# One-2-3-45/One-2-3-45

Measured on NVIDIA H100. Metric: sec/mesh end-to-end (256x256 in), lower is better.
Workload: dtype f16

## Files before the change

### one-2-3-45_b200/csrc/attention.cu

```cuda
#include <cuda_fp16.h>

#include "common.cuh"
#include "mma_sync.cuh"

namespace o2345 {
namespace {

__device__ __forceinline__ float ex2(float x) {
  float y;
  asm("ex2.approx.ftz.f32 %0, %1;" : "=f"(y) : "f"(x));
  return y;
}

constexpr int KT = 64;

template <int D, int DP, int NW>
__global__ void __launch_bounds__(32 * NW)
attention_kernel(const __half* __restrict__ q, const __half* __restrict__ k, const __half* __restrict__ v, int N, int H, int ld,
                 __half* __restrict__ out, int ldo, float scale_log2) {
  pdl_wait();
  pdl_trigger();
  constexpr int QT = 16 * NW, NT = 32 * NW;
  constexpr int LDQ = DP + 8, KS = DP / 16, NO = DP / 8;
  constexpr int STAGE = 2 * KT * LDQ;
  extern __shared__ __align__(16) __half smem_h[];
  __half* sQ = smem_h;
  __half* sKV = sQ + QT * LDQ;
  const int tid = threadIdx.x, warp = tid >> 5, lane = tid & 31, g = lane >> 2, t = lane & 3;
  const int bh = blockIdx.y, b = bh / H, h = bh % H;
  const int q0 = blockIdx.x * QT;
  const int64_t base = (int64_t)b * N * ld + (int64_t)h * D;
  constexpr int CH = D / 8;

  auto load_tile = [&](int stage, int k0) {
    __half* dK = sKV + stage * STAGE;
    __half* dV = dK + KT * LDQ;
    for (int i = tid; i < KT * CH; i += NT) {
      const int r = i / CH, c = i % CH;
      const bool in = k0 + r < N;
      const int64_t off = base + (int64_t)(in ? k0 + r : 0) * ld + 8 * c;
      const uint32_t ak = (uint32_t)__cvta_generic_to_shared(dK + r * LDQ + 8 * c), av = (uint32_t)__cvta_generic_to_shared(dV + r * LDQ + 8 * c);
      asm volatile("cp.async.cg.shared.global [%0], [%1], 16;" ::"r"(ak), "l"(k + off) : "memory");
      asm volatile("cp.async.cg.shared.global [%0], [%1], 16, %2;" ::"r"(av), "l"(v + off), "r"(in ? 16 : 0) : "memory");
    }
    asm volatile("cp.async.commit_group;" ::: "memory");
  };

  for (int i = tid; i < (QT * LDQ + 2 * STAGE) / 8; i += NT) reinterpret_cast<uint4*>(sQ)[i] = make_uint4(0, 0, 0, 0);
  __syncthreads();
  load_tile(0, 0);
  for (int i = tid; i < QT * CH; i += NT) {
    int r = i / CH, c = i % CH;
    if (q0 + r < N) *reinterpret_cast<uint4*>(sQ + r * LDQ + 8 * c) = *reinterpret_cast<const uint4*>(q + base + (int64_t)(q0 + r) * ld + 8 * c);
  }
  __syncthreads();
  uint32_t qa[KS][4];
#pragma unroll
  for (int kk = 0; kk < KS; ++kk) {
    const __half* p0 = sQ + (16 * warp + g) * LDQ + 16 * kk + 2 * t;
    qa[kk][0] = *reinterpret_cast<const uint32_t*>(p0);
    qa[kk][1] = *reinterpret_cast<const uint32_t*>(p0 + 8 * LDQ);
    qa[kk][2] = *reinterpret_cast<const uint32_t*>(p0 + 8);
    qa[kk][3] = *reinterpret_cast<const uint32_t*>(p0 + 8 * LDQ + 8);
  }
  float o[NO][4];
#pragma unroll
  for (int n = 0; n < NO; ++n) o[n][0] = o[n][1] = o[n][2] = o[n][3] = 0.f;
  float m0 = -1e30f, m1 = -1e30f;
  float ls[4] = {0.f, 0.f, 0.f, 0.f};

  int it = 0;
  for (int k0 = 0; k0 < N; k0 += KT, ++it) {
    asm volatile("cp.async.wait_group 0;" ::: "memory");
    __syncthreads();
    if (k0 + KT < N) load_tile((it + 1) & 1, k0 + KT);
    const __half* sK = sKV + (it & 1) * STAGE;
    const __half* sV = sK + KT * LDQ;
    float s[KT / 8][4];
#pragma unroll
    for (int j = 0; j < KT / 8; j += 2) {
      s[j][0] = s[j][1] = s[j][2] = s[j][3] = 0.f;
      s[j + 1][0] = s[j + 1][1] = s[j + 1][2] = s[j + 1][3] = 0.f;
#pragma unroll
      for (int kk = 0; kk < KS; ++kk) {
        uint32_t b0, b1, b2, b3;
        const uint32_t addr = (uint32_t)__cvta_generic_to_shared(sK + (8 * j + 8 * (lane >> 4) + (lane & 7)) * LDQ + 16 * kk + 8 * ((lane >> 3) & 1));
        asm volatile("ldmatrix.sync.aligned.m8n8.x4.shared.b16 {%0, %1, %2, %3}, [%4];" : "=r"(b0), "=r"(b1), "=r"(b2), "=r"(b3) : "r"(addr));
        mma16816(s[j], qa[kk], b0, b1);
        mma16816(s[j + 1], qa[kk], b2, b3);
      }
    }
    if (k0 + KT > N) {
#pragma unroll
      for (int j = 0; j < KT / 8; ++j) {
        const int key = k0 + 8 * j + 2 * t;
        if (key >= N) s[j][0] = -1e30f, s[j][2] = -1e30f;
        if (key + 1 >= N) s[j][1] = -1e30f, s[j][3] = -1e30f;
      }
    }
    float mx0 = -1e30f, mx1 = -1e30f;
#pragma unroll
    for (int j = 0; j < KT / 8; ++j) {
      mx0 = fmaxf(mx0, fmaxf(s[j][0], s[j][1]));
      mx1 = fmaxf(mx1, fmaxf(s[j][2], s[j][3]));
    }
    mx0 = fmaxf(mx0, __shfl_xor_sync(0xffffffffu, mx0, 1)), mx0 = fmaxf(mx0, __shfl_xor_sync(0xffffffffu, mx0, 2));
    mx1 = fmaxf(mx1, __shfl_xor_sync(0xffffffffu, mx1, 1)), mx1 = fmaxf(mx1, __shfl_xor_sync(0xffffffffu, mx1, 2));
    const float mn0 = fmaxf(m0, mx0), mn1 = fmaxf(m1, mx1);
    const float a0 = ex2((m0 - mn0) * scale_log2), a1 = ex2((m1 - mn1) * scale_log2);
    m0 = mn0, m1 = mn1;
    const float ms0 = -mn0 * scale_log2, ms1 = -mn1 * scale_log2;
#pragma unroll
    for (int n = 0; n < NO; ++n) o[n][0] *= a0, o[n][1] *= a0, o[n][2] *= a1, o[n][3] *= a1;
    ls[0] *= a0, ls[1] *= a0, ls[2] *= a1, ls[3] *= a1;
#pragma unroll
    for (int kk = 0; kk < KT / 16; ++kk) {
      const uint32_t pa[4] = {pack2(ex2(fmaf(s[2 * kk][0], scale_log2, ms0)), ex2(fmaf(s[2 * kk][1], scale_log2, ms0))),
                              pack2(ex2(fmaf(s[2 * kk][2], scale_log2, ms1)), ex2(fmaf(s[2 * kk][3], scale_log2, ms1))),
                              pack2(ex2(fmaf(s[2 * kk + 1][0], scale_log2, ms0)), ex2(fmaf(s[2 * kk + 1][1], scale_log2, ms0))),
                              pack2(ex2(fmaf(s[2 * kk + 1][2], scale_log2, ms1)), ex2(fmaf(s[2 * kk + 1][3], scale_log2, ms1)))};
      mma16816(ls, pa, 0x3C003C00u, 0x3C003C00u);
#pragma unroll
      for (int n = 0; n < NO; ++n) {
        uint32_t b0, b1;
        const uint32_t addr = (uint32_t)__cvta_generic_to_shared(sV + (16 * kk + (lane & 15)) * LDQ + 8 * n);
        asm volatile("ldmatrix.sync.aligned.m8n8.x2.trans.shared.b16 {%0, %1}, [%2];" : "=r"(b0), "=r"(b1) : "r"(addr));
        mma16816(o[n], pa, b0, b1);
      }
    }
  }
  const float l0 = ls[0], l1 = ls[2];
  float i0 = 1.f / l0, i1 = 1.f / l1;
  int row0 = q0 + 16 * warp + g, row1 = row0 + 8;
#pragma unroll
  for (int n = 0; n < NO; ++n) {
    int col = 8 * n + 2 * t;
    if (col < D) {
      if (row0 < N) *reinterpret_cast<uint32_t*>(out + ((int64_t)b * N + row0) * ldo + h * D + col) = pack2(o[n][0] * i0, o[n][1] * i0);
      if (row1 < N) *reinterpret_cast<uint32_t*>(out + ((int64_t)b * N + row1) * ldo + h * D + col) = pack2(o[n][2] * i1, o[n][3] * i1);
    }
  }
}

}
}

using namespace o2345;

extern "C" int o2345_attention_f16(const void* q, const void* k, const void* v, int B, int N, int H, int d, int ld, void* out,
                                   int ldo, float scale, o2345_stream_t stream) {
  O2345_CHECK_ARG(q && k && v && out, "null pointer");
  O2345_CHECK_ARG(B > 0 && N > 0 && H > 0 && (ld % 8) == 0 && (ldo % 2) == 0, "bad sizes");
  O2345_CHECK_ARG(d == 40 || d == 64 || d == 80 || d == 160, "head dim must be 40, 64, 80 or 160");
  O2345_CHECK_ARG(((uintptr_t)q % 16) == 0 && ((uintptr_t)k % 16) == 0 && ((uintptr_t)v % 16) == 0, "q/k/v must be 16-byte aligned");
  const int nw = N >= 512 ? 8 : 4;
  dim3 grid(cdiv(N, 16 * nw), B * H);
  float sl2 = scale * 1.4426950408889634f;
  cudaStream_t st = (cudaStream_t)stream;
  const __half *qh = (const __half*)q, *kh = (const __half*)k, *vh = (const __half*)v;
  auto smem = [&](int dp) { return (size_t)((16 * nw + 4 * KT) * (dp + 8)) * sizeof(__half); };
  static PerDeviceOnce attr;
  if (attr.need()) {
    O2345_CUDA(cudaFuncSetAttribute(attention_kernel<160, 160, 4>, cudaFuncAttributeMaxDynamicSharedMemorySize, (int)((64 + 4 * KT) * 168 * 2)));
    O2345_CUDA(cudaFuncSetAttribute(attention_kernel<160, 160, 8>, cudaFuncAttributeMaxDynamicSharedMemorySize, (int)((128 + 4 * KT) * 168 * 2)));
    O2345_CUDA(cudaFuncSetAttribute(attention_kernel<80, 80, 4>, cudaFuncAttributeMaxDynamicSharedMemorySize, (int)((64 + 4 * KT) * 88 * 2)));
    O2345_CUDA(cudaFuncSetAttribute(attention_kernel<80, 80, 8>, cudaFuncAttributeMaxDynamicSharedMemorySize, (int)((128 + 4 * KT) * 88 * 2)));
    O2345_CUDA(cudaFuncSetAttribute(attention_kernel<64, 64, 8>, cudaFuncAttributeMaxDynamicSharedMemorySize, (int)((128 + 4 * KT) * 72 * 2)));
  }
#define O2345_ATT(D_, DP_)                                                                                                        \
  do {                                                                                                                            \
    if (nw == 8)                                                                                                                  \
      O2345_CUDA(launch_pdl(attention_kernel<D_, DP_, 8>, dim3(grid), dim3(256), smem(DP_), st, qh, kh, vh, N, H, ld, (__half*)out, \
                            ldo, sl2));                                                                                           \
    else                                                                                                                          \
      O2345_CUDA(launch_pdl(attention_kernel<D_, DP_, 4>, dim3(grid), dim3(128), smem(DP_), st, qh, kh, vh, N, H, ld, (__half*)out, \
                            ldo, sl2));                                                                                           \
  } while (0)
  if (d == 40) O2345_ATT(40, 48);
  else if (d == 64) O2345_ATT(64, 64);
  else if (d == 80) O2345_ATT(80, 80);
  else if (d == 160) O2345_ATT(160, 160);
  else { set_error("o2345_attention_f16: head dim %d not built (40 / 64 / 80 / 160)", d); return O2345_EUNSUPPORTED; }
#undef O2345_ATT
  O2345_LAUNCH_CHECK();
  return O2345_OK;
}
```

### one-2-3-45_b200/csrc/wgmma.cuh

```cuda
#pragma once
#include <stdint.h>

namespace o2345 {
namespace wg {

__device__ __forceinline__ uint64_t desc_sw128(uint32_t saddr) {
  uint64_t d = 0;
  d |= (uint64_t)((saddr >> 4) & 0x3FFF);
  d |= (uint64_t)1 << 16;
  d |= (uint64_t)(1024 >> 4) << 32;
  d |= (uint64_t)1 << 62;
  return d;
}
__device__ __forceinline__ void fence() { asm volatile("wgmma.fence.sync.aligned;" ::: "memory"); }
__device__ __forceinline__ void commit() { asm volatile("wgmma.commit_group.sync.aligned;" ::: "memory"); }
template <int N>
__device__ __forceinline__ void wait() { asm volatile("wgmma.wait_group.sync.aligned %0;" ::"n"(N) : "memory"); }

template <int N>
__device__ __forceinline__ void mma_f16(float (&d)[N / 2], uint64_t adesc, uint64_t bdesc, int accumulate);

template <>
__device__ __forceinline__ void mma_f16<16>(float (&d)[8], uint64_t adesc, uint64_t bdesc, int accumulate) {
  asm volatile(
      "{\n\t.reg .pred p;\n\tsetp.ne.b32 p, %10, 0;\n\t"
      "wgmma.mma_async.sync.aligned.m64n16k16.f32.f16.f16 {%0, %1, %2, %3, %4, %5, %6, %7}, %8, %9, p, 1, 1, 0, 0;\n\t}"
      : "+f"(d[0]), "+f"(d[1]), "+f"(d[2]), "+f"(d[3]), "+f"(d[4]), "+f"(d[5]), "+f"(d[6]), "+f"(d[7])
      : "l"(adesc), "l"(bdesc), "r"(accumulate));
}

template <>
__device__ __forceinline__ void mma_f16<32>(float (&d)[16], uint64_t adesc, uint64_t bdesc, int accumulate) {
  asm volatile(
      "{\n\t.reg .pred p;\n\tsetp.ne.b32 p, %18, 0;\n\t"
      "wgmma.mma_async.sync.aligned.m64n32k16.f32.f16.f16 {%0, %1, %2, %3, %4, %5, %6, %7, %8, %9, %10, %11, %12, %13, %14, %15}, %16, %17, p, 1, 1, 0, 0;\n\t}"
      : "+f"(d[0]), "+f"(d[1]), "+f"(d[2]), "+f"(d[3]), "+f"(d[4]), "+f"(d[5]), "+f"(d[6]), "+f"(d[7]), "+f"(d[8]), "+f"(d[9]), "+f"(d[10]), "+f"(d[11]), "+f"(d[12]), "+f"(d[13]), "+f"(d[14]), "+f"(d[15])
      : "l"(adesc), "l"(bdesc), "r"(accumulate));
}

template <>
__device__ __forceinline__ void mma_f16<48>(float (&d)[24], uint64_t adesc, uint64_t bdesc, int accumulate) {
  asm volatile(
      "{\n\t.reg .pred p;\n\tsetp.ne.b32 p, %26, 0;\n\t"
      "wgmma.mma_async.sync.aligned.m64n48k16.f32.f16.f16 {%0, %1, %2, %3, %4, %5, %6, %7, %8, %9, %10, %11, %12, %13, %14, %15, %16, %17, %18, %19, %20, %21, %22, %23}, %24, %25, p, 1, 1, 0, 0;\n\t}"
      : "+f"(d[0]), "+f"(d[1]), "+f"(d[2]), "+f"(d[3]), "+f"(d[4]), "+f"(d[5]), "+f"(d[6]), "+f"(d[7]), "+f"(d[8]), "+f"(d[9]), "+f"(d[10]), "+f"(d[11]), "+f"(d[12]), "+f"(d[13]), "+f"(d[14]), "+f"(d[15]), "+f"(d[16]), "+f"(d[17]), "+f"(d[18]), "+f"(d[19]), "+f"(d[20]), "+f"(d[21]), "+f"(d[22]), "+f"(d[23])
      : "l"(adesc), "l"(bdesc), "r"(accumulate));
}

template <>
__device__ __forceinline__ void mma_f16<64>(float (&d)[32], uint64_t adesc, uint64_t bdesc, int accumulate) {
  asm volatile(
      "{\n\t.reg .pred p;\n\tsetp.ne.b32 p, %34, 0;\n\t"
      "wgmma.mma_async.sync.aligned.m64n64k16.f32.f16.f16 {%0, %1, %2, %3, %4, %5, %6, %7, %8, %9, %10, %11, %12, %13, %14, %15, %16, %17, %18, %19, %20, %21, %22, %23, %24, %25, %26, %27, %28, %29, %30, %31}, %32, %33, p, 1, 1, 0, 0;\n\t}"
      : "+f"(d[0]), "+f"(d[1]), "+f"(d[2]), "+f"(d[3]), "+f"(d[4]), "+f"(d[5]), "+f"(d[6]), "+f"(d[7]), "+f"(d[8]), "+f"(d[9]), "+f"(d[10]), "+f"(d[11]), "+f"(d[12]), "+f"(d[13]), "+f"(d[14]), "+f"(d[15]), "+f"(d[16]), "+f"(d[17]), "+f"(d[18]), "+f"(d[19]), "+f"(d[20]), "+f"(d[21]), "+f"(d[22]), "+f"(d[23]), "+f"(d[24]), "+f"(d[25]), "+f"(d[26]), "+f"(d[27]), "+f"(d[28]), "+f"(d[29]), "+f"(d[30]), "+f"(d[31])
      : "l"(adesc), "l"(bdesc), "r"(accumulate));
}

template <>
__device__ __forceinline__ void mma_f16<128>(float (&d)[64], uint64_t adesc, uint64_t bdesc, int accumulate) {
  asm volatile(
      "{\n\t.reg .pred p;\n\tsetp.ne.b32 p, %66, 0;\n\t"
      "wgmma.mma_async.sync.aligned.m64n128k16.f32.f16.f16 {%0, %1, %2, %3, %4, %5, %6, %7, %8, %9, %10, %11, %12, %13, %14, %15, %16, %17, %18, %19, %20, %21, %22, %23, %24, %25, %26, %27, %28, %29, %30, %31, %32, %33, %34, %35, %36, %37, %38, %39, %40, %41, %42, %43, %44, %45, %46, %47, %48, %49, %50, %51, %52, %53, %54, %55, %56, %57, %58, %59, %60, %61, %62, %63}, %64, %65, p, 1, 1, 0, 0;\n\t}"
      : "+f"(d[0]), "+f"(d[1]), "+f"(d[2]), "+f"(d[3]), "+f"(d[4]), "+f"(d[5]), "+f"(d[6]), "+f"(d[7]), "+f"(d[8]), "+f"(d[9]), "+f"(d[10]), "+f"(d[11]), "+f"(d[12]), "+f"(d[13]), "+f"(d[14]), "+f"(d[15]), "+f"(d[16]), "+f"(d[17]), "+f"(d[18]), "+f"(d[19]), "+f"(d[20]), "+f"(d[21]), "+f"(d[22]), "+f"(d[23]), "+f"(d[24]), "+f"(d[25]), "+f"(d[26]), "+f"(d[27]), "+f"(d[28]), "+f"(d[29]), "+f"(d[30]), "+f"(d[31]), "+f"(d[32]), "+f"(d[33]), "+f"(d[34]), "+f"(d[35]), "+f"(d[36]), "+f"(d[37]), "+f"(d[38]), "+f"(d[39]), "+f"(d[40]), "+f"(d[41]), "+f"(d[42]), "+f"(d[43]), "+f"(d[44]), "+f"(d[45]), "+f"(d[46]), "+f"(d[47]), "+f"(d[48]), "+f"(d[49]), "+f"(d[50]), "+f"(d[51]), "+f"(d[52]), "+f"(d[53]), "+f"(d[54]), "+f"(d[55]), "+f"(d[56]), "+f"(d[57]), "+f"(d[58]), "+f"(d[59]), "+f"(d[60]), "+f"(d[61]), "+f"(d[62]), "+f"(d[63])
      : "l"(adesc), "l"(bdesc), "r"(accumulate));
}

template <>
__device__ __forceinline__ void mma_f16<160>(float (&d)[80], uint64_t adesc, uint64_t bdesc, int accumulate) {
  asm volatile(
      "{\n\t.reg .pred p;\n\tsetp.ne.b32 p, %82, 0;\n\t"
      "wgmma.mma_async.sync.aligned.m64n160k16.f32.f16.f16 {%0, %1, %2, %3, %4, %5, %6, %7, %8, %9, %10, %11, %12, %13, %14, %15, %16, %17, %18, %19, %20, %21, %22, %23, %24, %25, %26, %27, %28, %29, %30, %31, %32, %33, %34, %35, %36, %37, %38, %39, %40, %41, %42, %43, %44, %45, %46, %47, %48, %49, %50, %51, %52, %53, %54, %55, %56, %57, %58, %59, %60, %61, %62, %63, %64, %65, %66, %67, %68, %69, %70, %71, %72, %73, %74, %75, %76, %77, %78, %79}, %80, %81, p, 1, 1, 0, 0;\n\t}"
      : "+f"(d[0]), "+f"(d[1]), "+f"(d[2]), "+f"(d[3]), "+f"(d[4]), "+f"(d[5]), "+f"(d[6]), "+f"(d[7]), "+f"(d[8]), "+f"(d[9]), "+f"(d[10]), "+f"(d[11]), "+f"(d[12]), "+f"(d[13]), "+f"(d[14]), "+f"(d[15]), "+f"(d[16]), "+f"(d[17]), "+f"(d[18]), "+f"(d[19]), "+f"(d[20]), "+f"(d[21]), "+f"(d[22]), "+f"(d[23]), "+f"(d[24]), "+f"(d[25]), "+f"(d[26]), "+f"(d[27]), "+f"(d[28]), "+f"(d[29]), "+f"(d[30]), "+f"(d[31]), "+f"(d[32]), "+f"(d[33]), "+f"(d[34]), "+f"(d[35]), "+f"(d[36]), "+f"(d[37]), "+f"(d[38]), "+f"(d[39]), "+f"(d[40]), "+f"(d[41]), "+f"(d[42]), "+f"(d[43]), "+f"(d[44]), "+f"(d[45]), "+f"(d[46]), "+f"(d[47]), "+f"(d[48]), "+f"(d[49]), "+f"(d[50]), "+f"(d[51]), "+f"(d[52]), "+f"(d[53]), "+f"(d[54]), "+f"(d[55]), "+f"(d[56]), "+f"(d[57]), "+f"(d[58]), "+f"(d[59]), "+f"(d[60]), "+f"(d[61]), "+f"(d[62]), "+f"(d[63]), "+f"(d[64]), "+f"(d[65]), "+f"(d[66]), "+f"(d[67]), "+f"(d[68]), "+f"(d[69]), "+f"(d[70]), "+f"(d[71]), "+f"(d[72]), "+f"(d[73]), "+f"(d[74]), "+f"(d[75]), "+f"(d[76]), "+f"(d[77]), "+f"(d[78]), "+f"(d[79])
      : "l"(adesc), "l"(bdesc), "r"(accumulate));
}

template <>
__device__ __forceinline__ void mma_f16<256>(float (&d)[128], uint64_t adesc, uint64_t bdesc, int accumulate) {
  asm volatile(
      "{\n\t.reg .pred p;\n\tsetp.ne.b32 p, %130, 0;\n\t"
      "wgmma.mma_async.sync.aligned.m64n256k16.f32.f16.f16 {%0, %1, %2, %3, %4, %5, %6, %7, %8, %9, %10, %11, %12, %13, %14, %15, %16, %17, %18, %19, %20, %21, %22, %23, %24, %25, %26, %27, %28, %29, %30, %31, %32, %33, %34, %35, %36, %37, %38, %39, %40, %41, %42, %43, %44, %45, %46, %47, %48, %49, %50, %51, %52, %53, %54, %55, %56, %57, %58, %59, %60, %61, %62, %63, %64, %65, %66, %67, %68, %69, %70, %71, %72, %73, %74, %75, %76, %77, %78, %79, %80, %81, %82, %83, %84, %85, %86, %87, %88, %89, %90, %91, %92, %93, %94, %95, %96, %97, %98, %99, %100, %101, %102, %103, %104, %105, %106, %107, %108, %109, %110, %111, %112, %113, %114, %115, %116, %117, %118, %119, %120, %121, %122, %123, %124, %125, %126, %127}, %128, %129, p, 1, 1, 0, 0;\n\t}"
      : "+f"(d[0]), "+f"(d[1]), "+f"(d[2]), "+f"(d[3]), "+f"(d[4]), "+f"(d[5]), "+f"(d[6]), "+f"(d[7]), "+f"(d[8]), "+f"(d[9]), "+f"(d[10]), "+f"(d[11]), "+f"(d[12]), "+f"(d[13]), "+f"(d[14]), "+f"(d[15]), "+f"(d[16]), "+f"(d[17]), "+f"(d[18]), "+f"(d[19]), "+f"(d[20]), "+f"(d[21]), "+f"(d[22]), "+f"(d[23]), "+f"(d[24]), "+f"(d[25]), "+f"(d[26]), "+f"(d[27]), "+f"(d[28]), "+f"(d[29]), "+f"(d[30]), "+f"(d[31]), "+f"(d[32]), "+f"(d[33]), "+f"(d[34]), "+f"(d[35]), "+f"(d[36]), "+f"(d[37]), "+f"(d[38]), "+f"(d[39]), "+f"(d[40]), "+f"(d[41]), "+f"(d[42]), "+f"(d[43]), "+f"(d[44]), "+f"(d[45]), "+f"(d[46]), "+f"(d[47]), "+f"(d[48]), "+f"(d[49]), "+f"(d[50]), "+f"(d[51]), "+f"(d[52]), "+f"(d[53]), "+f"(d[54]), "+f"(d[55]), "+f"(d[56]), "+f"(d[57]), "+f"(d[58]), "+f"(d[59]), "+f"(d[60]), "+f"(d[61]), "+f"(d[62]), "+f"(d[63]), "+f"(d[64]), "+f"(d[65]), "+f"(d[66]), "+f"(d[67]), "+f"(d[68]), "+f"(d[69]), "+f"(d[70]), "+f"(d[71]), "+f"(d[72]), "+f"(d[73]), "+f"(d[74]), "+f"(d[75]), "+f"(d[76]), "+f"(d[77]), "+f"(d[78]), "+f"(d[79]), "+f"(d[80]), "+f"(d[81]), "+f"(d[82]), "+f"(d[83]), "+f"(d[84]), "+f"(d[85]), "+f"(d[86]), "+f"(d[87]), "+f"(d[88]), "+f"(d[89]), "+f"(d[90]), "+f"(d[91]), "+f"(d[92]), "+f"(d[93]), "+f"(d[94]), "+f"(d[95]), "+f"(d[96]), "+f"(d[97]), "+f"(d[98]), "+f"(d[99]), "+f"(d[100]), "+f"(d[101]), "+f"(d[102]), "+f"(d[103]), "+f"(d[104]), "+f"(d[105]), "+f"(d[106]), "+f"(d[107]), "+f"(d[108]), "+f"(d[109]), "+f"(d[110]), "+f"(d[111]), "+f"(d[112]), "+f"(d[113]), "+f"(d[114]), "+f"(d[115]), "+f"(d[116]), "+f"(d[117]), "+f"(d[118]), "+f"(d[119]), "+f"(d[120]), "+f"(d[121]), "+f"(d[122]), "+f"(d[123]), "+f"(d[124]), "+f"(d[125]), "+f"(d[126]), "+f"(d[127])
      : "l"(adesc), "l"(bdesc), "r"(accumulate));
}

}
}
```

Measured before the change: 2.505.

## Add wgmma-based flash attention kernel for head dim 40

Adds a Hopper warpgroup-MMA attention kernel for head dimension 40. It uses a 4-stage cp.async K/V pipeline with core-matrix shared layouts, and overlaps the next tile's QK^T wgmma with the current tile's PV wgmma. The row sum is folded into the PV matmul by appending a ones column to V and a masking column to Q/K, which also masks out-of-range keys. This targets the mma.sync tensor-core throughput limit for the d=40 attention in the diffusion UNet, at the cost of more complex descriptor and layout logic and a higher risk of correctness bugs.

```diff
diff --git a/one-2-3-45_b200/csrc/attention.cu b/one-2-3-45_b200/csrc/attention.cu
--- a/one-2-3-45_b200/csrc/attention.cu
+++ b/one-2-3-45_b200/csrc/attention.cu
@@ -2,6 +2,7 @@
 
 #include "common.cuh"
 #include "mma_sync.cuh"
+#include "wgmma.cuh"
 
 namespace o2345 {
 namespace {
@@ -16,7 +17,7 @@
 
 template <int D, int DP, int NW>
 __global__ void __launch_bounds__(32 * NW)
-attention_kernel(const __half* __restrict__ q, const __half* __restrict__ k, const __half* __restrict__ v, int N, int H, int ld,
+attention_mma_kernel(const __half* __restrict__ q, const __half* __restrict__ k, const __half* __restrict__ v, int N, int H, int ld,
                  __half* __restrict__ out, int ldo, float scale_log2) {
   pdl_wait();
   pdl_trigger();
@@ -142,10 +143,175 @@
   }
 }
 
+template <int N>
+__device__ __forceinline__ void fence_regs(float (&r)[N]) {
+#pragma unroll
+  for (int i = 0; i < N; ++i) asm volatile("" : "+f"(r[i])::"memory");
+}
+
+constexpr int STAGES = 4;
+
+__device__ __forceinline__ uint32_t cm_off(int r, int c, int C) { return (uint32_t)((r >> 3) * (C * 128) + c * 128 + (r & 7) * 16); }
+
+template <int D, int NWG>
+struct AttCfg {
+  static constexpr int CH = D / 8;
+  static constexpr int CK = (CH + 2) / 2 * 2;
+  static constexpr int DV = D + 8;
+  static constexpr int CV = DV / 8;
+  static constexpr int QT = 64 * NWG;
+  static constexpr int QB = QT * CK * 16, KB = KT * CK * 16, VB = KT * CV * 16, SB = KB + VB;
+  static constexpr int SMEM = QB + STAGES * SB;
+};
+
+template <int D, int NWG>
+__global__ void __launch_bounds__(128 * NWG)
+attention_wgmma_kernel(const __half* __restrict__ q, const __half* __restrict__ k, const __half* __restrict__ v, int N, int H, int ld,
+                 __half* __restrict__ out, int ldo, float scale_log2) {
+  pdl_wait();
+  pdl_trigger();
+  using C = AttCfg<D, NWG>;
+  constexpr int CH = C::CH, CK = C::CK, CV = C::CV, DV = C::DV, NT = 128 * NWG;
+  extern __shared__ __align__(128) uint8_t smem[];
+  const uint32_t sbase = (uint32_t)__cvta_generic_to_shared(smem);
+  const int tid = threadIdx.x, warp = tid >> 5, lane = tid & 31, g = lane >> 2, t = lane & 3, wg = warp >> 2;
+  const int bh = blockIdx.y, b = bh / H, h = bh % H;
+  const int q0 = blockIdx.x * C::QT;
+  const int64_t base = (int64_t)b * N * ld + (int64_t)h * D;
+  const int nt = (N + KT - 1) / KT;
+
+  for (int i = tid; i < STAGES * KT; i += NT) {
+    uint8_t* st = smem + C::QB + (i / KT) * C::SB;
+    const int r = i % KT;
+    *reinterpret_cast<uint4*>(st + C::KB + cm_off(r, CH, CV)) = make_uint4(0x3C003C00u, 0x3C003C00u, 0x3C003C00u, 0x3C003C00u);
+#pragma unroll
+    for (int c = CH; c < CK; ++c) *reinterpret_cast<uint4*>(st + cm_off(r, c, CK)) = make_uint4(0, 0, 0, 0);
+  }
+  for (int i = tid; i < C::QT; i += NT)
+#pragma unroll
+    for (int c = CH; c < CK; ++c) *reinterpret_cast<uint4*>(smem + cm_off(i, c, CK)) = make_uint4(c == CH ? 0x3C00u : 0u, 0, 0, 0);
+
+  auto copy_rows = [&](uint32_t dst, int C_, const __half* src, int r0, int rows) {
+    for (int i = tid; i < rows * CH; i += NT) {
+      const int rr = i & 7, c = (i >> 3) % CH, r = (i >> 3) / CH * 8 + rr;
+      const bool in = r0 + r < N;
+      const __half* p = src + base + (int64_t)(in ? r0 + r : 0) * ld + 8 * c;
+      asm volatile("cp.async.cg.shared.global [%0], [%1], 16, %2;" ::"r"(dst + cm_off(r, c, C_)), "l"(p), "r"(in ? 16 : 0) : "memory");
+    }
+  };
+  auto load_tile = [&](int j) {
+    const uint32_t st = sbase + C::QB + (j % STAGES) * C::SB;
+    if (j < nt) {
+      copy_rows(st, CK, k, j * KT, KT);
+      copy_rows(st + C::KB, CV, v, j * KT, KT);
+    }
+    asm volatile("cp.async.commit_group;" ::: "memory");
+    if (j == nt - 1)
+      for (int r = N - j * KT + tid; r < KT; r += NT)
+        *reinterpret_cast<uint4*>(smem + (st - sbase) + cm_off(r, CH, CK)) = make_uint4(0xFC00u, 0, 0, 0);
+  };
+  copy_rows(sbase, CK, q, q0, C::QT);
+  load_tile(0);
+  load_tile(1);
+  load_tile(2);
+
+  const uint64_t qdesc = wg::desc_plain(sbase + wg * 64 * CK * 16, 128, CK * 128);
+  auto issue_s = [&](float (&s)[32], int j) {
+    const uint32_t st = sbase + C::QB + (j % STAGES) * C::SB;
+    fence_regs(s);
+    wg::fence();
+#pragma unroll
+    for (int kk = 0; kk < CK / 2; ++kk) wg::mma_f16<64>(s, qdesc + 16 * kk, wg::desc_plain(st + 256 * kk, 128, CK * 128), kk);
+    wg::commit();
+  };
+  float s[32], o[DV / 2];
+#pragma unroll
+  for (int i = 0; i < DV / 2; ++i) o[i] = 0.f;
+  float m0 = -1e30f, m1 = -1e30f;
+  float a0 = 1.f, a1 = 1.f;
+  uint32_t pa[KT / 16][4];
+
+  auto softmax = [&]() {
+    float mx0 = -1e30f, mx1 = -1e30f;
+#pragma unroll
+    for (int n = 0; n < KT / 8; ++n) {
+      mx0 = fmaxf(mx0, fmaxf(s[4 * n], s[4 * n + 1]));
+      mx1 = fmaxf(mx1, fmaxf(s[4 * n + 2], s[4 * n + 3]));
+    }
+    mx0 = fmaxf(mx0, __shfl_xor_sync(0xffffffffu, mx0, 1)), mx0 = fmaxf(mx0, __shfl_xor_sync(0xffffffffu, mx0, 2));
+    mx1 = fmaxf(mx1, __shfl_xor_sync(0xffffffffu, mx1, 1)), mx1 = fmaxf(mx1, __shfl_xor_sync(0xffffffffu, mx1, 2));
+    const float mn0 = fmaxf(m0, mx0), mn1 = fmaxf(m1, mx1);
+    a0 = ex2((m0 - mn0) * scale_log2), a1 = ex2((m1 - mn1) * scale_log2);
+    m0 = mn0, m1 = mn1;
+    const float ms0 = -mn0 * scale_log2, ms1 = -mn1 * scale_log2;
+#pragma unroll
+    for (int n = 0; n < KT / 8; ++n) {
+      s[4 * n] = ex2(fmaf(s[4 * n], scale_log2, ms0)), s[4 * n + 1] = ex2(fmaf(s[4 * n + 1], scale_log2, ms0));
+      s[4 * n + 2] = ex2(fmaf(s[4 * n + 2], scale_log2, ms1)), s[4 * n + 3] = ex2(fmaf(s[4 * n + 3], scale_log2, ms1));
+    }
+  };
+  auto to_pa = [&]() {
+#pragma unroll
+    for (int kk = 0; kk < KT / 16; ++kk) {
+      const float* c0 = s + 8 * kk;
+      pa[kk][0] = pack2(c0[0], c0[1]), pa[kk][1] = pack2(c0[2], c0[3]), pa[kk][2] = pack2(c0[4], c0[5]), pa[kk][3] = pack2(c0[6], c0[7]);
+    }
+  };
+
+  asm volatile("cp.async.wait_group 2;" ::: "memory");
+  asm volatile("fence.proxy.async.shared::cta;" ::: "memory");
+  __syncthreads();
+  issue_s(s, 0);
+  wg::wait<0>();
+  fence_regs(s);
+  softmax();
+  to_pa();
+  auto issue_pv = [&](int j) {
+    const uint32_t sv = sbase + C::QB + (j % STAGES) * C::SB + C::KB;
+    wg::fence();
+#pragma unroll
+    for (int kk = 0; kk < KT / 16; ++kk) wg::mma_f16_rs_mn<DV>(o, pa[kk], wg::desc_plain(sv + kk * 2 * CV * 128, CV * 128, 128));
+    wg::commit();
+  };
+  for (int j = 0; j + 1 < nt; ++j) {
+    asm volatile("cp.async.wait_group 1;" ::: "memory");
+    asm volatile("fence.proxy.async.shared::cta;" ::: "memory");
+    __syncthreads();
+    load_tile(j + 3);
+    issue_s(s, j + 1);
+    issue_pv(j);
+    wg::wait<1>();
+    fence_regs(s);
+    softmax();
+    wg::wait<0>();
+    fence_regs(o);
+#pragma unroll
+    for (int n = 0; n < DV / 8; ++n) o[4 * n] *= a0, o[4 * n + 1] *= a0, o[4 * n + 2] *= a1, o[4 * n + 3] *= a1;
+    fence_regs(o);
+    to_pa();
+  }
+  issue_pv(nt - 1);
+  wg::wait<0>();
+  fence_regs(o);
+
+  const float l0 = __shfl_sync(0xffffffffu, o[4 * (D / 8)], lane & ~3), l1 = __shfl_sync(0xffffffffu, o[4 * (D / 8) + 2], lane & ~3);
+  const float i0 = 1.f / l0, i1 = 1.f / l1;
+  const int row0 = q0 + 64 * wg + 16 * (warp & 3) + g, row1 = row0 + 8;
+#pragma unroll
+  for (int n = 0; n < CH; ++n) {
+    const int col = 8 * n + 2 * t;
+    if (row0 < N) *reinterpret_cast<uint32_t*>(out + ((int64_t)b * N + row0) * ldo + h * D + col) = pack2(o[4 * n] * i0, o[4 * n + 1] * i0);
+    if (row1 < N) *reinterpret_cast<uint32_t*>(out + ((int64_t)b * N + row1) * ldo + h * D + col) = pack2(o[4 * n + 2] * i1, o[4 * n + 3] * i1);
+  }
+}
+
+
 }
 }
 
 using namespace o2345;
+
+constexpr int WG_LONG = 4;
 
 extern "C" int o2345_attention_f16(const void* q, const void* k, const void* v, int B, int N, int H, int d, int ld, void* out,
                                    int ldo, float scale, o2345_stream_t stream) {
@@ -153,31 +319,43 @@
   O2345_CHECK_ARG(B > 0 && N > 0 && H > 0 && (ld % 8) == 0 && (ldo % 2) == 0, "bad sizes");
   O2345_CHECK_ARG(d == 40 || d == 64 || d == 80 || d == 160, "head dim must be 40, 64, 80 or 160");
   O2345_CHECK_ARG(((uintptr_t)q % 16) == 0 && ((uintptr_t)k % 16) == 0 && ((uintptr_t)v % 16) == 0, "q/k/v must be 16-byte aligned");
-  const int nw = N >= 512 ? 8 : 4;
-  dim3 grid(cdiv(N, 16 * nw), B * H);
   float sl2 = scale * 1.4426950408889634f;
   cudaStream_t st = (cudaStream_t)stream;
   const __half *qh = (const __half*)q, *kh = (const __half*)k, *vh = (const __half*)v;
-  auto smem = [&](int dp) { return (size_t)((16 * nw + 4 * KT) * (dp + 8)) * sizeof(__half); };
+  __half* oh = (__half*)out;
   static PerDeviceOnce attr;
   if (attr.need()) {
-    O2345_CUDA(cudaFuncSetAttribute(attention_kernel<160, 160, 4>, cudaFuncAttributeMaxDynamicSharedMemorySize, (int)((64 + 4 * KT) * 168 * 2)));
-    O2345_CUDA(cudaFuncSetAttribute(attention_kernel<160, 160, 8>, cudaFuncAttributeMaxDynamicSharedMemorySize, (int)((128 + 4 * KT) * 168 * 2)));
-    O2345_CUDA(cudaFuncSetAttribute(attention_kernel<80, 80, 4>, cudaFuncAttributeMaxDynamicSharedMemorySize, (int)((64 + 4 * KT) * 88 * 2)));
-    O2345_CUDA(cudaFuncSetAttribute(attention_kernel<80, 80, 8>, cudaFuncAttributeMaxDynamicSharedMemorySize, (int)((128 + 4 * KT) * 88 * 2)));
-    O2345_CUDA(cudaFuncSetAttribute(attention_kernel<64, 64, 8>, cudaFuncAttributeMaxDynamicSharedMemorySize, (int)((128 + 4 * KT) * 72 * 2)));
-  }
+    O2345_CUDA(cudaFuncSetAttribute(attention_mma_kernel<160, 160, 4>, cudaFuncAttributeMaxDynamicSharedMemorySize, (int)((64 + 4 * KT) * 168 * 2)));
+    O2345_CUDA(cudaFuncSetAttribute(attention_mma_kernel<160, 160, 8>, cudaFuncAttributeMaxDynamicSharedMemorySize, (int)((128 + 4 * KT) * 168 * 2)));
+    O2345_CUDA(cudaFuncSetAttribute(attention_mma_kernel<80, 80, 4>, cudaFuncAttributeMaxDynamicSharedMemorySize, (int)((64 + 4 * KT) * 88 * 2)));
+    O2345_CUDA(cudaFuncSetAttribute(attention_mma_kernel<80, 80, 8>, cudaFuncAttributeMaxDynamicSharedMemorySize, (int)((128 + 4 * KT) * 88 * 2)));
+    O2345_CUDA(cudaFuncSetAttribute(attention_mma_kernel<64, 64, 8>, cudaFuncAttributeMaxDynamicSharedMemorySize, (int)((128 + 4 * KT) * 72 * 2)));
+    O2345_CUDA(cudaFuncSetAttribute(attention_wgmma_kernel<40, 1>, cudaFuncAttributeMaxDynamicSharedMemorySize, AttCfg<40, 1>::SMEM));
+    O2345_CUDA(cudaFuncSetAttribute(attention_wgmma_kernel<40, WG_LONG>, cudaFuncAttributeMaxDynamicSharedMemorySize, AttCfg<40, WG_LONG>::SMEM));
+  }
+  if (d == 40) {
+    if (N >= 512)
+      O2345_CUDA(launch_pdl(attention_wgmma_kernel<40, WG_LONG>, dim3(cdiv(N, 64 * WG_LONG), B * H), dim3(128 * WG_LONG),
+                            (size_t)AttCfg<40, WG_LONG>::SMEM, st, qh, kh, vh, N, H, ld, oh, ldo, sl2));
+    else
+      O2345_CUDA(launch_pdl(attention_wgmma_kernel<40, 1>, dim3(cdiv(N, 64), B * H), dim3(128), (size_t)AttCfg<40, 1>::SMEM, st, qh,
+                            kh, vh, N, H, ld, oh, ldo, sl2));
+    O2345_LAUNCH_CHECK();
+    return O2345_OK;
+  }
+  const int nw = N >= 512 ? 8 : 4;
+  dim3 grid(cdiv(N, 16 * nw), B * H);
+  auto smem = [&](int dp) { return (size_t)((16 * nw + 4 * KT) * (dp + 8)) * sizeof(__half); };
 #define O2345_ATT(D_, DP_)                                                                                                        \
   do {                                                                                                                            \
     if (nw == 8)                                                                                                                  \
-      O2345_CUDA(launch_pdl(attention_kernel<D_, DP_, 8>, dim3(grid), dim3(256), smem(DP_), st, qh, kh, vh, N, H, ld, (__half*)out, \
+      O2345_CUDA(launch_pdl(attention_mma_kernel<D_, DP_, 8>, dim3(grid), dim3(256), smem(DP_), st, qh, kh, vh, N, H, ld, oh,     \
                             ldo, sl2));                                                                                           \
     else                                                                                                                          \
-      O2345_CUDA(launch_pdl(attention_kernel<D_, DP_, 4>, dim3(grid), dim3(128), smem(DP_), st, qh, kh, vh, N, H, ld, (__half*)out, \
+      O2345_CUDA(launch_pdl(attention_mma_kernel<D_, DP_, 4>, dim3(grid), dim3(128), smem(DP_), st, qh, kh, vh, N, H, ld, oh,     \
                             ldo, sl2));                                                                                           \
   } while (0)
-  if (d == 40) O2345_ATT(40, 48);
-  else if (d == 64) O2345_ATT(64, 64);
+  if (d == 64) O2345_ATT(64, 64);
   else if (d == 80) O2345_ATT(80, 80);
   else if (d == 160) O2345_ATT(160, 160);
   else { set_error("o2345_attention_f16: head dim %d not built (40 / 64 / 80 / 160)", d); return O2345_EUNSUPPORTED; }
diff --git a/one-2-3-45_b200/csrc/wgmma.cuh b/one-2-3-45_b200/csrc/wgmma.cuh
--- a/one-2-3-45_b200/csrc/wgmma.cuh
+++ b/one-2-3-45_b200/csrc/wgmma.cuh
@@ -10,6 +10,13 @@
   d |= (uint64_t)1 << 16;
   d |= (uint64_t)(1024 >> 4) << 32;
   d |= (uint64_t)1 << 62;
+  return d;
+}
+__device__ __forceinline__ uint64_t desc_plain(uint32_t saddr, uint32_t lbo, uint32_t sbo) {
+  uint64_t d = 0;
+  d |= (uint64_t)((saddr >> 4) & 0x3FFF);
+  d |= (uint64_t)((lbo >> 4) & 0x3FFF) << 16;
+  d |= (uint64_t)((sbo >> 4) & 0x3FFF) << 32;
   return d;
 }
 __device__ __forceinline__ void fence() { asm volatile("wgmma.fence.sync.aligned;" ::: "memory"); }
@@ -83,5 +90,44 @@
       : "l"(adesc), "l"(bdesc), "r"(accumulate));
 }
 
+template <int N>
+__device__ __forceinline__ void mma_f16_rs_mn(float (&d)[N / 2], const uint32_t (&a)[4], uint64_t bdesc);
+
+template <>
+__device__ __forceinline__ void mma_f16_rs_mn<48>(float (&d)[24], const uint32_t (&a)[4], uint64_t bdesc) {
+  asm volatile(
+      "{\n\t.reg .pred p;\n\tsetp.ne.b32 p, 1, 0;\n\t"
+      "wgmma.mma_async.sync.aligned.m64n48k16.f32.f16.f16 {%0, %1, %2, %3, %4, %5, %6, %7, %8, %9, %10, %11, %12, %13, %14, %15, %16, %17, %18, %19, %20, %21, %22, %23}, {%24, %25, %26, %27}, %28, p, 1, 1, 1;\n\t}"
+      : "+f"(d[0]), "+f"(d[1]), "+f"(d[2]), "+f"(d[3]), "+f"(d[4]), "+f"(d[5]), "+f"(d[6]), "+f"(d[7]), "+f"(d[8]), "+f"(d[9]), "+f"(d[10]), "+f"(d[11]), "+f"(d[12]), "+f"(d[13]), "+f"(d[14]), "+f"(d[15]), "+f"(d[16]), "+f"(d[17]), "+f"(d[18]), "+f"(d[19]), "+f"(d[20]), "+f"(d[21]), "+f"(d[22]), "+f"(d[23])
+      : "r"(a[0]), "r"(a[1]), "r"(a[2]), "r"(a[3]), "l"(bdesc));
+}
+
+template <>
+__device__ __forceinline__ void mma_f16_rs_mn<72>(float (&d)[36], const uint32_t (&a)[4], uint64_t bdesc) {
+  asm volatile(
+      "{\n\t.reg .pred p;\n\tsetp.ne.b32 p, 1, 0;\n\t"
+      "wgmma.mma_async.sync.aligned.m64n72k16.f32.f16.f16 {%0, %1, %2, %3, %4, %5, %6, %7, %8, %9, %10, %11, %12, %13, %14, %15, %16, %17, %18, %19, %20, %21, %22, %23, %24, %25, %26, %27, %28, %29, %30, %31, %32, %33, %34, %35}, {%36, %37, %38, %39}, %40, p, 1, 1, 1;\n\t}"
+      : "+f"(d[0]), "+f"(d[1]), "+f"(d[2]), "+f"(d[3]), "+f"(d[4]), "+f"(d[5]), "+f"(d[6]), "+f"(d[7]), "+f"(d[8]), "+f"(d[9]), "+f"(d[10]), "+f"(d[11]), "+f"(d[12]), "+f"(d[13]), "+f"(d[14]), "+f"(d[15]), "+f"(d[16]), "+f"(d[17]), "+f"(d[18]), "+f"(d[19]), "+f"(d[20]), "+f"(d[21]), "+f"(d[22]), "+f"(d[23]), "+f"(d[24]), "+f"(d[25]), "+f"(d[26]), "+f"(d[27]), "+f"(d[28]), "+f"(d[29]), "+f"(d[30]), "+f"(d[31]), "+f"(d[32]), "+f"(d[33]), "+f"(d[34]), "+f"(d[35])
+      : "r"(a[0]), "r"(a[1]), "r"(a[2]), "r"(a[3]), "l"(bdesc));
+}
+
+template <>
+__device__ __forceinline__ void mma_f16_rs_mn<88>(float (&d)[44], const uint32_t (&a)[4], uint64_t bdesc) {
+  asm volatile(
+      "{\n\t.reg .pred p;\n\tsetp.ne.b32 p, 1, 0;\n\t"
+      "wgmma.mma_async.sync.aligned.m64n88k16.f32.f16.f16 {%0, %1, %2, %3, %4, %5, %6, %7, %8, %9, %10, %11, %12, %13, %14, %15, %16, %17, %18, %19, %20, %21, %22, %23, %24, %25, %26, %27, %28, %29, %30, %31, %32, %33, %34, %35, %36, %37, %38, %39, %40, %41, %42, %43}, {%44, %45, %46, %47}, %48, p, 1, 1, 1;\n\t}"
+      : "+f"(d[0]), "+f"(d[1]), "+f"(d[2]), "+f"(d[3]), "+f"(d[4]), "+f"(d[5]), "+f"(d[6]), "+f"(d[7]), "+f"(d[8]), "+f"(d[9]), "+f"(d[10]), "+f"(d[11]), "+f"(d[12]), "+f"(d[13]), "+f"(d[14]), "+f"(d[15]), "+f"(d[16]), "+f"(d[17]), "+f"(d[18]), "+f"(d[19]), "+f"(d[20]), "+f"(d[21]), "+f"(d[22]), "+f"(d[23]), "+f"(d[24]), "+f"(d[25]), "+f"(d[26]), "+f"(d[27]), "+f"(d[28]), "+f"(d[29]), "+f"(d[30]), "+f"(d[31]), "+f"(d[32]), "+f"(d[33]), "+f"(d[34]), "+f"(d[35]), "+f"(d[36]), "+f"(d[37]), "+f"(d[38]), "+f"(d[39]), "+f"(d[40]), "+f"(d[41]), "+f"(d[42]), "+f"(d[43])
+      : "r"(a[0]), "r"(a[1]), "r"(a[2]), "r"(a[3]), "l"(bdesc));
+}
+
+template <>
+__device__ __forceinline__ void mma_f16_rs_mn<168>(float (&d)[84], const uint32_t (&a)[4], uint64_t bdesc) {
+  asm volatile(
+      "{\n\t.reg .pred p;\n\tsetp.ne.b32 p, 1, 0;\n\t"
+      "wgmma.mma_async.sync.aligned.m64n168k16.f32.f16.f16 {%0, %1, %2, %3, %4, %5, %6, %7, %8, %9, %10, %11, %12, %13, %14, %15, %16, %17, %18, %19, %20, %21, %22, %23, %24, %25, %26, %27, %28, %29, %30, %31, %32, %33, %34, %35, %36, %37, %38, %39, %40, %41, %42, %43, %44, %45, %46, %47, %48, %49, %50, %51, %52, %53, %54, %55, %56, %57, %58, %59, %60, %61, %62, %63, %64, %65, %66, %67, %68, %69, %70, %71, %72, %73, %74, %75, %76, %77, %78, %79, %80, %81, %82, %83}, {%84, %85, %86, %87}, %88, p, 1, 1, 1;\n\t}"
+      : "+f"(d[0]), "+f"(d[1]), "+f"(d[2]), "+f"(d[3]), "+f"(d[4]), "+f"(d[5]), "+f"(d[6]), "+f"(d[7]), "+f"(d[8]), "+f"(d[9]), "+f"(d[10]), "+f"(d[11]), "+f"(d[12]), "+f"(d[13]), "+f"(d[14]), "+f"(d[15]), "+f"(d[16]), "+f"(d[17]), "+f"(d[18]), "+f"(d[19]), "+f"(d[20]), "+f"(d[21]), "+f"(d[22]), "+f"(d[23]), "+f"(d[24]), "+f"(d[25]), "+f"(d[26]), "+f"(d[27]), "+f"(d[28]), "+f"(d[29]), "+f"(d[30]), "+f"(d[31]), "+f"(d[32]), "+f"(d[33]), "+f"(d[34]), "+f"(d[35]), "+f"(d[36]), "+f"(d[37]), "+f"(d[38]), "+f"(d[39]), "+f"(d[40]), "+f"(d[41]), "+f"(d[42]), "+f"(d[43]), "+f"(d[44]), "+f"(d[45]), "+f"(d[46]), "+f"(d[47]), "+f"(d[48]), "+f"(d[49]), "+f"(d[50]), "+f"(d[51]), "+f"(d[52]), "+f"(d[53]), "+f"(d[54]), "+f"(d[55]), "+f"(d[56]), "+f"(d[57]), "+f"(d[58]), "+f"(d[59]), "+f"(d[60]), "+f"(d[61]), "+f"(d[62]), "+f"(d[63]), "+f"(d[64]), "+f"(d[65]), "+f"(d[66]), "+f"(d[67]), "+f"(d[68]), "+f"(d[69]), "+f"(d[70]), "+f"(d[71]), "+f"(d[72]), "+f"(d[73]), "+f"(d[74]), "+f"(d[75]), "+f"(d[76]), "+f"(d[77]), "+f"(d[78]), "+f"(d[79]), "+f"(d[80]), "+f"(d[81]), "+f"(d[82]), "+f"(d[83])
+      : "r"(a[0]), "r"(a[1]), "r"(a[2]), "r"(a[3]), "l"(bdesc));
+}
+
 }
 }
```

Result: no change. 2.500 (median of 6 runs) (-0.2%).
